# masapasa/qcpinn-convection-diffusion-qiskit

Hardware: AMD Instinct MI355X
Metric: collocation-points/sec (PDE+BC+IC loss step), 4-qubit cascade (higher is better)
Workload: dtype f32

## Files before the change

qcpinn-convection-diffusion-qiskit_amd/csrc/qc_circuit_reg_kernels.h:

```cpp
#pragma once
#include "qc_gates.h"
#include "qc_internal.h"

#include <stdlib.h>

#include <utility>

namespace {

template <int AB>
__device__ __forceinline__ bool qc_flag(int rt) {
  if constexpr (AB < 0) return rt != 0;
  else return AB != 0;
}

template <class T>
__device__ __forceinline__ const T* qc_launder(const T* p) {
  asm volatile("" : "+s"(p));
  return p;
}
template <class T>
__device__ __forceinline__ const __attribute__((address_space(4))) T* qc_const(const T* p) {
  return (const __attribute__((address_space(4))) T*)qc_launder(p);
}
// ... 11 lines not shown
__device__ __forceinline__ int64_t qc_opaque_s(int64_t v) {
  asm volatile("" : "+s"(v));
  return v;
}
__device__ __forceinline__ int qc_opaque_v(int v) {
  asm volatile("" : "+v"(v));
  return v;
}

template <int NQ>
struct DynProg {
  static constexpr int N = NQ;
  static constexpr bool lead_rx = true;
  __device__ static __forceinline__ int lead_slot(const QcGate* __restrict__ prog, int w) { return prog[w].slot; }
  template <int AB = -1, bool PIN = false>
  __device__ static __forceinline__ void fwd(SV<NQ> (&v)[1], const QcGate* __restrict__ prog,
                                             const QcTrig* __restrict__ trig, const float* __restrict__ umat,
                                             int n_gates, int absorb) {
    for (int g = qc_flag<AB>(absorb) ? NQ : 0; g < n_gates; ++g) {
      const QcGate gt = prog[g];
      const QcTrig tr = trig[g];
      qc_apply_gate<NQ, 1, false>(v, gt, tr.c, tr.s, umat);
    }
  }
  template <int AB = -1>
  __device__ static __forceinline__ void bwd(SV<NQ> (&cl)[2], const QcGate* __restrict__ prog,
                                             const QcTrig* __restrict__ trig, const float* __restrict__ umat,
                                             int n_gates, float* __restrict__ acc_wave, int lane, int absorb) {
    const int g_first = qc_flag<AB>(absorb) ? NQ : 0;
    for (int g = n_gates - 1; g >= g_first; --g) {
      const QcGate gt = prog[g];
      const QcTrig tr = trig[g];
      if (gt.op != QC_U4 && gt.slot >= 0) {
        const float gr = qc_wave_sum_to_lane63(qc_gate_grad<NQ>(cl[1], cl[0], gt));
        if (lane == 63) acc_wave[gt.slot] += gr;
      }
      qc_apply_gate<NQ, 2, true>(cl, gt, tr.c, tr.s, umat);
    }
  }
};

struct SGate {
  int op, ba, bb, slot;
};

template <int NQ, int K, bool ADJ, int OP, int BA, int BB, int SLOT>
__device__ __forceinline__ void qc_static_gate(SV<NQ> (&v)[K], const float c, const float s_in) {
  const float s = ADJ ? -s_in : s_in;
#pragma unroll
  for (int q = 0; q < K; ++q) {
    if constexpr (OP == QC_RX) g_rx<NQ, BA>(v[q], c, s);
    else if constexpr (OP == QC_RY) g_ry<NQ, BA>(v[q], c, s);
    else if constexpr (OP == QC_RZ) g_rz<NQ, BA>(v[q], c, s);
    else if constexpr (OP == QC_H) g_h<NQ, BA>(v[q]);
    else if constexpr (OP == QC_CNOT) g_cnot<NQ, BA, BB>(v[q]);
    else if constexpr (OP == QC_CRX) g_crx<NQ, BA, BB>(v[q], c, s);
    else if constexpr (OP == QC_CRZ) g_crz<NQ, BA, BB>(v[q], c, s);
  }
}

template <int NQ, int OP, int BA, int BB>
__device__ __forceinline__ float qc_static_grad(const SV<NQ>& lam, const SV<NQ>& chi) {
  if constexpr (OP == QC_RX) return ip_x<NQ, BA>(lam, chi);
  else if constexpr (OP == QC_RY) return ip_y<NQ, BA>(lam, chi);
  else if constexpr (OP == QC_RZ) return ip_z<NQ, BA>(lam, chi);
  else if constexpr (OP == QC_CRX) return ip_cx<NQ, BA, BB>(lam, chi);
  else if constexpr (OP == QC_CRZ) return ip_cz<NQ, BA, BB>(lam, chi);
// ... 33 lines not shown
    (load_one<Is, AB>(t, trig), ...);
    __builtin_amdgcn_sched_barrier(0);
  }
  static constexpr bool is_diag(int i) { return i >= 0 && i < SP::G && (SP::g[i].op == QC_RZ || SP::g[i].op == QC_CRZ); }
  static constexpr int run_begin(int i) { while (is_diag(i - 1)) --i; return i; }
  static constexpr int run_end(int i) { while (is_diag(i)) ++i; return i; }
  static constexpr bool fused(int i) { return is_diag(i) && run_end(i) - run_begin(i) >= 2; }
  static constexpr int run_ordinal(int i) {
    int r = 0;
    for (int g = 0; g < run_begin(i);) {
      if (!is_diag(g)) { ++g; continue; }
      const int e = run_end(g);
      if (e - g >= 2) ++r;
      g = e;
    }
    return r;
  }
  static_assert(run_ordinal(SP::G) <= QC_MAX_DIAG_RUNS, "more fused diagonal runs than the host records (qc_find_diag_runs)");
  template <int I, bool ADJ, int K, bool PIN = true>
  __device__ static __forceinline__ void apply_table(SV<N> (&v)[K], const QcTrig* __restrict__ trig) {
    constexpr int off = SP::G + run_ordinal(I) * (1 << N);
    auto run = [&](auto tab) {
#pragma unroll
      for (int k = 0; k < (1 << N); ++k) {
        const float dr = tab[k].c, di = ADJ ? -tab[k].s : tab[k].s;
#pragma unroll
        for (int q = 0; q < K; ++q) v[q].a[k] = qc_cmul(dr, di, v[q].a[k]);
      }
    };
    if constexpr (PIN) run(qc_const_at(trig, v[0]) + off);
    else run(trig + off);
  }
  template <int H, int E>
  __device__ static __forceinline__ void run_grads(const QcPk<(1 << N)>& t, float (&gacc)[SP::P > 0 ? SP::P : 1]) {
    if constexpr (H < E) {
      constexpr SGate g = SP::g[H];
      constexpr bool ctl = g.op == QC_CRZ;
      constexpr int tb = ctl ? g.bb : g.ba;
      constexpr int cb = ctl ? g.ba : -1;
      qf2 a2 = {0.f, 0.f};
#pragma unroll
      for (int j = 0; j < (1 << (N - 1)); ++j) {
        if (cb >= 1 && !((j >> (cb >= 1 ? cb - 1 : 0)) & 1)) continue;
        if (tb >= 1 && ((j >> (tb >= 1 ? tb - 1 : 0)) & 1)) a2 -= t.p[j];
        else a2 += t.p[j];
      }
      const float acc = tb == 0 ? a2.x - a2.y : (cb == 0 ? a2.y : a2.x + a2.y);
      if constexpr (g.slot >= 0) gacc[g.slot] += qc_wave_sum_to_lane63(acc);
      run_grads<H + 1, E>(t, gacc);
    }
  }
  template <int I, int K, bool ADJ, bool PIN = true>
  __device__ static __forceinline__ void gate(SV<N> (&v)[K], const Trig& t, const float* __restrict__ umat) {
    constexpr SGate g = SP::g[I];
    if constexpr (g.op == QC_U4) {
      constexpr int off = (g.slot * 2 + (ADJ ? 1 : 0)) * 32;
      if constexpr (PIN) {
        const CMat u = qc_const_at(umat, v[0]) + off;
#pragma unroll
        for (int q = 0; q < K; ++q) g_u4<N, g.ba, g.bb>(v[q], u);
      } else {
#pragma unroll
        for (int q = 0; q < K; ++q) g_u4<N, g.ba, g.bb>(v[q], umat + off);
      }
    } else {
      qc_static_gate<N, K, ADJ, g.op, g.ba, g.bb, g.slot>(v, t.c[I], t.s[I]);
    }
  }
  template <int I, int AB, bool PIN>
  __device__ static __forceinline__ void fwd_one(SV<N> (&v)[1], const Trig& t, const float* __restrict__ umat,
                                                 int absorb, const QcTrig* __restrict__ trig) {
    if constexpr (I < N) {
      if (qc_flag<AB>(absorb)) return;
    }
    if constexpr (fused(I)) {
      if constexpr (I == run_begin(I)) {
        apply_table<I, false, 1, PIN>(v, trig);
        __builtin_amdgcn_sched_barrier(0);
      }
    } else {
      gate<I, 1, false, PIN>(v, t, umat);
      __builtin_amdgcn_sched_barrier(0);
    }
  }
  template <int AB, bool PIN, int... Is>
  __device__ static __forceinline__ void fwd_all(SV<N> (&v)[1], const Trig& t, const float* __restrict__ umat,
                                                 int absorb, const QcTrig* __restrict__ trig,
                                                 std::integer_sequence<int, Is...>) {
    (fwd_one<Is, AB, PIN>(v, t, umat, absorb, trig), ...);
  }
  template <int AB = -1, bool PIN = false>
  __device__ static __forceinline__ void fwd(SV<N> (&v)[1], const QcGate* __restrict__, const QcTrig* __restrict__ trig,
                                             const float* __restrict__ umat, int, int absorb) {
    Trig t;
    if constexpr (PIN) load_all<AB>(t, qc_const(trig), std::make_integer_sequence<int, SP::G>{});
    else load_all<AB>(t, trig, std::make_integer_sequence<int, SP::G>{});
    fwd_all<AB, PIN>(v, t, umat, absorb, trig, std::make_integer_sequence<int, SP::G>{});
  }
  template <int J, int AB>
  __device__ static __forceinline__ void bwd_one(SV<N> (&cl)[2], const Trig& t, const float* __restrict__ umat,
                                                 float (&gacc)[SP::P > 0 ? SP::P : 1], int absorb,
                                                 const QcTrig* __restrict__ trig) {
    constexpr int I = SP::G - 1 - J;
    constexpr SGate g = SP::g[I];
    if constexpr (I < N) {
      if (qc_flag<AB>(absorb)) return;
    }
    if constexpr (fused(I)) {
      if constexpr (I == run_end(I) - 1) {
        QcPk<(1 << N)> tk;
#pragma unroll
        for (int k = 0; k < (1 << N); ++k) {
          const qf2 m = cl[1].a[k] * qc_swp(cl[0].a[k]);
          tk[k] = m.x - m.y;
        }
        run_grads<run_begin(I), run_end(I)>(tk, gacc);
        apply_table<I, true, 2>(cl, trig);
        __builtin_amdgcn_sched_barrier(0);
      }
    } else {
      if constexpr (g.op != QC_U4 && g.slot >= 0)
        gacc[g.slot] += qc_wave_sum_to_lane63(qc_static_grad<N, g.op, g.ba, g.bb>(cl[1], cl[0]));
      gate<I, 2, true>(cl, t, umat);
      __builtin_amdgcn_sched_barrier(0);
    }
  }
  template <int AB, int... Js>
  __device__ static __forceinline__ void bwd_all(SV<N> (&cl)[2], const Trig& t, const float* __restrict__ umat,
                                                 float (&gacc)[SP::P > 0 ? SP::P : 1], int absorb,
                                                 const QcTrig* __restrict__ trig, std::integer_sequence<int, Js...>) {
    (bwd_one<Js, AB>(cl, t, umat, gacc, absorb, trig), ...);
  }
  template <int AB = -1>
  __device__ static __forceinline__ void bwd(SV<N> (&cl)[2], const QcGate* __restrict__, const QcTrig* __restrict__ trig,
                                             const float* __restrict__ umat, int, float* __restrict__ acc_wave,
                                             int lane, int absorb) {
    float gacc[SP::P > 0 ? SP::P : 1];
#pragma unroll
    for (int k = 0; k < (SP::P > 0 ? SP::P : 1); ++k) gacc[k] = 0.f;
    Trig t;
    load_all<AB>(t, qc_const(trig), std::make_integer_sequence<int, SP::G>{});
    bwd_all<AB>(cl, t, umat, gacc, absorb, trig, std::make_integer_sequence<int, SP::G>{});
    const int k0 = qc_opaque_v(0);
    const bool last = qc_opaque_v(lane) == 63;
#pragma unroll
    for (int k = 0; k < SP::P; ++k)
      if (last) acc_wave[k0 + k] += gacc[k];
  }
};

template <int AB = -1>
__device__ __forceinline__ void qc_wire_sincos(float& c, float& s, const float* __restrict__ a, int64_t B, int64_t p, int w,
                                               const QcTrig* __restrict__ trig, int absorb) {
  const float h = 0.5f * (a[(int64_t)w * B + p] + (qc_flag<AB>(absorb) ? trig[w].th : 0.f));
  sincosf(h, &s, &c);
// ... 111 lines not shown
  SV<N> cl[2];
  {
    SV<N> v[1];
    build_channel<N, AB>(v[0], 0, angles, B, pc, ampl, trig, absorb);
    PG::template fwd<AB, true>(v, prog, trig, umat, n_gates, absorb);
    cl[0] = v[0];
  }
  float qb[N];
#pragma unroll
  for (int w = 0; w < N; ++w) qb[w] = live ? cot[(int64_t)w * B + pc] : 0.f;
  {
    QcPk<(1 << N)> d;
    qc_sign_sums<N>(d, qb);
#pragma unroll
    for (int k = 0; k < (1 << N); ++k) cl[1].a[k] = qc_dup(d[k]) * cl[0].a[k];
  }
  PG::template bwd<AB>(cl, prog, trig, umat, n_gates, smem + wave * n_params, lane, absorb);
  float T[N];
  if (ampl) {
#pragma unroll
    for (int w = 0; w < N; ++w) T[w] = 2.f * cl[1].a[w].x;
  } else {
    QcPk<(1 << N)> Q0, Q1, Q2;
    channel_series<N, AB>(Q0, Q1, Q2, 0, qc_launder(angles), B, pc, trig, absorb);
    qc_embed_ip<N>(T, cl[1], Q0);
  }
  if (live) {
#pragma unroll
    for (int w = 0; w < N; ++w) d_angles[(int64_t)w * B + p] = T[w];
  }
  if (qc_flag<AB>(absorb)) {
#pragma unroll
    for (int w = 0; w < N; ++w) {
      const float tot = qc_wave_sum_to_lane63(live ? T[w] : 0.f);
      if (lane == 63) smem[wave * n_params + (AB < 0 ? prog[w].slot : PG::lead_slot(prog, w))] += tot;
    }
  }
  __syncthreads();
  const int64_t tile = (int64_t)bid * WPB + wave;
  if (tile * 64 < B)
    for (int i = lane; i < n_params; i += 64) part[(row0 + tile) * part_stride + i] = smem[wave * n_params + i];
}

template <class PG>
__global__ void __launch_bounds__(256) k_value_bwd(const QcGate* __restrict__ prog, const QcTrig* __restrict__ trig,
                                                   const float* __restrict__ umat, int n_gates, int n_params,
                                                   const float* __restrict__ angles, const float* __restrict__ cot,
                                                   float* __restrict__ d_angles, float* __restrict__ part,
                                                   int64_t part_stride, int64_t row0, int64_t B, int amp) {
  k_value_bwd_body<PG, 4>(blockIdx.x, prog, trig, umat, n_gates, n_params, angles, cot, d_angles, part, part_stride, row0, B, amp);
}

template <int A2>
__device__ __forceinline__ int64_t qc_chi_pair(int ch, int k, int64_t p) {
  return ((((p >> 6) * 6 + ch) * (A2 / 2) + k) << 6) | (p & 63);
}
template <int N>
__device__ __forceinline__ void qc_chi_write(float* __restrict__ chi_store, int ch, int64_t p, const SV<N>& v) {
  qf2* cs = reinterpret_cast<qf2*>(chi_store);
#pragma unroll
  for (int k = 0; k < (1 << N); ++k) cs[qc_chi_pair<(2 << N)>(ch, k, p)] = v.a[k];
}
template <int N>
__device__ __forceinline__ void qc_chi_read(SV<N>& v, const float* __restrict__ chi_store, int ch, int64_t p) {
  const qf2* cs = reinterpret_cast<const qf2*>(chi_store);
#pragma unroll
  for (int k = 0; k < (1 << N); ++k) v.a[k] = cs[qc_chi_pair<(2 << N)>(ch, k, p)];
// ... 178 lines not shown
    } else if (ch <= 3) {
      qc_pull_ip1<N>(T, cl[1], da);
  #pragma unroll
      for (int w = 0; w < N; ++w) buf[(0 * N + w) * 64 + lane] = T[w];
      qc_pull_ip0<N>(T, cl[1]);
  #pragma unroll
      for (int w = 0; w < N; ++w) buf[(1 * N + w) * 64 + lane] = T[w];
    } else {
      qc_pull_ip2<N>(T, cl[1], da, dda);
  #pragma unroll
      for (int w = 0; w < N; ++w) buf[(0 * N + w) * 64 + lane] = T[w];
      qc_pull_ip1<N>(T, cl[1], da);
  #pragma unroll
      for (int w = 0; w < N; ++w) buf[(1 * N + w) * 64 + lane] = 2.f * T[w];
      qc_pull_ip0<N>(T, cl[1]);
  #pragma unroll
      for (int w = 0; w < N; ++w) buf[(2 * N + w) * 64 + lane] = T[w];
    }
    __syncthreads();
    auto at = [&](int wv, int slot, int w) { return s_chi[((wv * 3 + slot) * N + w) * 64 + lane]; };
  #pragma unroll
    for (int w = 0; w < N; ++w) {
      float r;
      if (ch == 0)
        r = ((at(0, 0, w) + at(1, 0, w)) + (at(2, 0, w) + at(3, 0, w))) + (at(4, 0, w) + at(5, 0, w));
      else if (ch == 1)
        r = at(1, 1, w);
      else if (ch <= 3)
        r = at(ch, 1, w) + at(ch + 2, 1, w);
      else
        r = at(ch, 2, w);
      if (live) abar[((int64_t)ch * N + w) * B + p] = r;
      if ((amp >> 1) && ch == 0) {
        const float tot = qc_wave_sum_to_lane63(live ? r : 0.f);
        if (lane == 63) s_acc[prog[w].slot] += tot;
      }
    }
    __syncthreads();
  }
  for (int i = threadIdx.x; i < n_params; i += 384) {
    float s = 0.f;
#pragma unroll
    for (int wv = 0; wv < 6; ++wv) s += s_acc[wv * n_params + i];
    part[(row0 + bid) * part_stride + i] = s;
  }
}

template <class PG, bool LOAD>
__global__ void __launch_bounds__(384, QC_JB_WAVES) k_jets_bwd(const QcGate* __restrict__ prog, const QcTrig* __restrict__ trig,
                                                  const float* __restrict__ umat, int n_gates, int n_params,
                                                  const float* __restrict__ ajets, const float* __restrict__ qbar,
                                                  float* __restrict__ abar, float* __restrict__ part,
                                                  int64_t part_stride, int64_t row0, int64_t B,
                                                  const float* __restrict__ chi_store, int amp) {
  k_jets_bwd_body<PG, LOAD>(blockIdx.x, prog, trig, umat, n_gates, n_params, ajets, qbar, abar, part, part_stride, row0, B, chi_store, amp);
}

struct QcPartRow {
  float* row;
  int n_params;
};
template <class PG, bool ABSORB, class ROW>
__device__ __forceinline__ void k_jets_bwd2_body(const int64_t bid, const QcGate* __restrict__ prog, const QcTrig* __restrict__ trig,
                                                   const float* __restrict__ umat, int n_gates, int n_params,
                                                   const float* __restrict__ ajets, const float* __restrict__ qbar,
                                                   float* __restrict__ abar, const ROW row_of, int64_t B,
                                                   const float* __restrict__ chi_store) {
// ... 103 lines not shown
      for (int w = 0; w < N; ++w) t_own[w] += T[w];
    } else if (ch <= 3) {
      qc_pull_ip1<N>(T, cl[1], da);
#pragma unroll
      for (int w = 0; w < N; ++w) t_own[w] += T[w];
      qc_pull_ip0<N>(T, cl[1]);
#pragma unroll
      for (int w = 0; w < N; ++w) t_a1[w] = T[w];
    } else {
      qc_pull_ip2<N>(T, cl[1], da, dda);
#pragma unroll
      for (int w = 0; w < N; ++w) t_own[w] += T[w];
      qc_pull_ip1<N>(T, cl[1], da);
#pragma unroll
      for (int w = 0; w < N; ++w) t_a1[w] = fmaf(2.f, T[w], t_a1[w]);
      qc_pull_ip0<N>(T, cl[1]);
      if (live) {
#pragma unroll
        for (int w = 0; w < N; ++w) abar[((int64_t)ch * N + w) * Bq + p] = T[w];
      }
    }
  }
  const int wt = wvf();
  if (live) {
#pragma unroll
    for (int w = 0; w < N; ++w) abar[((int64_t)(wt == 0 ? 1 : wt + 1) * N + w) * B + p] = t_a1[w];
  }
  if (wt != 0) {
#pragma unroll
    for (int w = 0; w < N; ++w) s_t0[((wt - 1) * N + w) * 64 + lane] = t_own[w];
  }
  __syncthreads();
  if (wt == 0) {
#pragma unroll
    for (int w = 0; w < N; ++w) {
      const float r = (t_own[w] + s_t0[w * 64 + lane]) + s_t0[(N + w) * 64 + lane];
      if (live) abar[(int64_t)w * B + p] = r;
      if constexpr (ABSORB) {
        const float tot = qc_wave_sum_to_lane63(live ? r : 0.f);
        if (lane == 63) s_acc[PG::lead_slot(prog, w)] += tot;
      }
    }
  }
  __syncthreads();
  const QcPartRow pr = row_of();
  float* __restrict__ row = pr.row;
  for (int i = threadIdx.x; i < pr.n_params; i += 192) row[i] = (s_acc[i] + s_acc[pr.n_params + i]) + s_acc[2 * pr.n_params + i];
}

template <class PG>
__global__ void __launch_bounds__(384) k_circ_fwd_both(const QcGate* __restrict__ prog, const QcTrig* __restrict__ trig,
                                                       const float* __restrict__ umat, int n_gates,
                                                       const float* __restrict__ ajets, float* __restrict__ qjets, int64_t Br,
                                                       float* __restrict__ chi_store, const float* __restrict__ angles,
                                                       float* __restrict__ expval, int64_t Bv, int amp, int n_val) {
  if ((int)blockIdx.x >= n_val) k_jets_fwd_body<PG>(blockIdx.x - n_val, prog, trig, umat, n_gates, ajets, qjets, Br, chi_store, amp);
  else k_value_fwd_body<PG, 6>(blockIdx.x, prog, trig, umat, n_gates, angles, expval, Bv, amp);
}

template <class PG>
__global__ void __launch_bounds__(384, QC_JB_WAVES) k_circ_bwd_both(
    const QcGate* __restrict__ prog, const QcTrig* __restrict__ trig, const float* __restrict__ umat, int n_gates, int n_params,
    const float* __restrict__ ajets, const float* __restrict__ qbar, float* __restrict__ abar, int64_t row0_r, int64_t Br,
    const float* __restrict__ chi_store, const float* __restrict__ angles, const float* __restrict__ cot,
    float* __restrict__ d_angles, int64_t row0_v, int64_t Bv, float* __restrict__ part, int64_t part_stride, int amp, int n_val) {
  if ((int)blockIdx.x >= n_val)
    k_jets_bwd_body<PG, true>(blockIdx.x - n_val, prog, trig, umat, n_gates, n_params, ajets, qbar, abar, part, part_stride, row0_r, Br,
                              chi_store, amp);
  else
    k_value_bwd_body<PG, 6>(blockIdx.x, prog, trig, umat, n_gates, n_params, angles, cot, d_angles, part, part_stride,
                            row0_v, Bv, amp);
}

struct QcBwdResArgs {
// ... 155 lines not shown
```

qcpinn-convection-diffusion-qiskit_amd/csrc/qc_common.h:

```cpp
#pragma once
#include <hip/hip_runtime.h>
#include <stdint.h>

#include "qc_types.h"

#define QC_NCH 6

#define QC_WAVE 64

static inline int qc_ceil_div(int64_t a, int64_t b) { return (int)((a + b - 1) / b); }

__host__ __device__ inline bool qc_is_diag_op(int op) { return op == 2  || op == 6 ; }

struct QcDiagRuns {
  int n;
  int g0[QC_MAX_DIAG_RUNS], g1[QC_MAX_DIAG_RUNS];
  const int* list;
};

inline void qc_find_diag_runs(qc_program* pg) {
  pg->n_diag_runs = 0;
  pg->d_diag_list = nullptr;
  if (pg->n_qubits > 5) return;
  for (int g = 0; g < pg->n_gates;) {
// ... 143 lines not shown
    }
    QcTrig t = {dr, di, 0.f, 0.f};
    trig[n_gates + r * A + k] = t;
  }
}

__device__ __forceinline__ float qc_wave_sum_to_lane63(float v) {
  v += __builtin_bit_cast(float, __builtin_amdgcn_update_dpp(0, __builtin_bit_cast(int, v), 0xB1, 0xF, 0xF, true));
  v += __builtin_bit_cast(float, __builtin_amdgcn_update_dpp(0, __builtin_bit_cast(int, v), 0x4E, 0xF, 0xF, true));
  v += __builtin_bit_cast(float, __builtin_amdgcn_update_dpp(0, __builtin_bit_cast(int, v), 0x141, 0xF, 0xF, true));
  v += __builtin_bit_cast(float, __builtin_amdgcn_update_dpp(0, __builtin_bit_cast(int, v), 0x140, 0xF, 0xF, true));
  v += __builtin_bit_cast(float, __builtin_amdgcn_update_dpp(0, __builtin_bit_cast(int, v), 0x142, 0xA, 0xF, false));
  v += __builtin_bit_cast(float, __builtin_amdgcn_update_dpp(0, __builtin_bit_cast(int, v), 0x143, 0xC, 0xF, false));
  return v;
}

template <int NV>
__device__ __forceinline__ void qc_wave_sum_multi_to_lane63(float (&v)[NV]) {
#define QC_DPP_STEP_(CTRL)                                                                                       \
  _Pragma("unroll") for (int k = 0; k < NV; ++k)                                                                 \
    v[k] += __builtin_bit_cast(float, __builtin_amdgcn_update_dpp(0, __builtin_bit_cast(int, v[k]), CTRL, 0xF, 0xF, true));
  QC_DPP_STEP_(0xB1) QC_DPP_STEP_(0x4E) QC_DPP_STEP_(0x141) QC_DPP_STEP_(0x140)
#undef QC_DPP_STEP_
#pragma unroll
  for (int k = 0; k < NV; ++k) asm volatile("" : "+v"(v[k]));
  asm volatile("s_nop 1");
#pragma unroll
  for (int k = 0; k < NV; ++k) asm volatile("v_add_f32_dpp %0, %0, %0 row_bcast:15 row_mask:0xa bank_mask:0xf" : "+v"(v[k]));
  if constexpr (NV < 3) asm volatile("s_nop 1");
#pragma unroll
  for (int k = 0; k < NV; ++k) asm volatile("v_add_f32_dpp %0, %0, %0 row_bcast:31 row_mask:0xc bank_mask:0xf" : "+v"(v[k]));
}

__device__ __forceinline__ float qc_wave_sum(float v) {
  v = qc_wave_sum_to_lane63(v);
  return __builtin_bit_cast(float, __builtin_amdgcn_readlane(__builtin_bit_cast(int, v), 63));
}
```

qcpinn-convection-diffusion-qiskit_amd/csrc/qc_mlp.hip:

```cpp
#include "qc_internal.h"
#include "qc_philox.h"
#include <tuple>

namespace {

__device__ __forceinline__ float qc_tanh(float x) {
  const float e = __expf(2.f * x);
  return 1.f - 2.f * __builtin_amdgcn_rcpf(e + 1.f);
}

typedef float mf2 __attribute__((ext_vector_type(2)));
__device__ __forceinline__ mf2 m_dup(const float a) { return (mf2){a, a}; }
__device__ __forceinline__ mf2 m_fma(const mf2 a, const mf2 b, const mf2 c) { return __builtin_elementwise_fma(a, b, c); }

__device__ __forceinline__ float analytic_u(float t, float x, float y) {
  const float dx = x - 0.5f, dy = y - 0.5f;
  return expf(-100.f * (dx * dx + dy * dy)) * expf(-t);
}
__device__ __forceinline__ float analytic_r(float t, float x, float y, float D, float vx, float vy) {
  const float u = analytic_u(t, x, y);
  const float dx = x - 0.5f, dy = y - 0.5f;
  const float ut = -u, ux = -200.f * dx * u, uy = -200.f * dy * u;
  const float uxx = (40000.f * dx * dx - 400.f) * u;
  const float uyy = (40000.f * dy * dy - 400.f) * u;
// ... 531 lines not shown

template <int N, int NCH>
__device__ __forceinline__ void post_cotangents(float (&gb)[NCH], float& gw4, const float (&g)[NCH],
                                                const float (&ub)[NCH], const float z, const float w4) {
  const float d1 = 1.f - z * z;
  gw4 = ub[0] * z;
  gb[0] = ub[0] * d1;
  if constexpr (NCH == 6) {
    const float d2 = -2.f * z * d1;
    const float d3 = -2.f * (d1 * d1 + z * d2);
    const float gx2 = g[2] * g[2], gy2 = g[3] * g[3];
    const float lin = ub[1] * g[1] + ub[2] * g[2] + ub[3] * g[3];
    gw4 += d1 * lin + ub[4] * (d2 * gx2 + d1 * g[4]) + ub[5] * (d2 * gy2 + d1 * g[5]);
    gb[0] += d2 * lin + ub[4] * (d3 * gx2 + d2 * g[4]) + ub[5] * (d3 * gy2 + d2 * g[5]);
    gb[1] = ub[1] * d1;
    gb[2] = ub[2] * d1 + 2.f * ub[4] * d2 * g[2];
    gb[3] = ub[3] * d1 + 2.f * ub[5] * d2 * g[3];
    gb[4] = ub[4] * d1;
    gb[5] = ub[5] * d1;
  }
#pragma unroll
  for (int c = 0; c < NCH; ++c) gb[c] *= w4;
}

template <int NCH>
__device__ __forceinline__ void expand_ub(float (&ub)[NCH], float ub0, float gsc, const QcPde& pde) {
  ub[0] = ub0;
  if constexpr (NCH == 6) {
    ub[1] = gsc * pde.c_t;
    ub[2] = gsc * pde.c_x;
    ub[3] = gsc * pde.c_y;
    ub[4] = -pde.d_xx * gsc;
    ub[5] = -pde.d_yy * gsc;
  }
}

__device__ __forceinline__ void learn_coefs(float (&cf)[QC_COEF_N], const float* __restrict__ prm, const QcLayout& L,
                                            const float (&base)[QC_COEF_N], const float (&scale)[QC_COEF_N]) {
  const float* __restrict__ pk = prm + (L.NP - QC_COEF_N);
#pragma unroll
  for (int k = 0; k < QC_COEF_N; ++k) cf[k] = fmaf(scale[k], pk[k], base[k]);
}
__device__ __forceinline__ void learn_columns(float* __restrict__ row, const QcLayout& L, const QcLearn* lr, const int z,
                                              const float (&scale)[QC_COEF_N], const float (&cf)[QC_COEF_N], const float gsc,
                                              const float (&u)[6], const int lane, const bool tile0) {
  float gv[QC_COEF_N] = {gsc * u[0], gsc * u[1], gsc * u[2], gsc * u[3], -gsc * u[4], -gsc * u[5], gsc * (u[0] * u[0] * u[0])};
  qc_wave_sum_multi_to_lane63<QC_COEF_N>(gv);
  if (lane == 63) {
#pragma unroll
    for (int k = 0; k < QC_COEF_N; ++k) row[L.NP - QC_COEF_N + k] = scale[k] == 0.f ? 0.f : scale[k] * gv[k];
    if (tile0) {
      float* hist = (&lr->hist)[z];
      const QcOptState* st = (&lr->st)[z];
      if (hist != nullptr && st != nullptr) {
        const int hi = st->step - st->hist_base;
        if (hi >= 0 && hi < (&lr->hist_cap)[z]) {
#pragma unroll
          for (int k = 0; k < QC_COEF_N; ++k) hist[(int64_t)hi * QC_COEF_N + k] = cf[k];
        }
      }
    }
  }
}
__device__ __forceinline__ int learn_late() {
  int z = 0;
#if defined(__HIP_DEVICE_COMPILE__)
// ... 639 lines not shown
  }
}

constexpr int QC_POST_VALUE_TPB = 1;

template <int N>
struct QcPostW {
  template <int K>
  struct Blk { static constexpr int count = K; float w3[K][N], b3[K], w4[K]; };
};
template <int N, int K>
__device__ __forceinline__ void post_blk_load(typename QcPostW<N>::template Blk<K>& w, const float* __restrict__ W3,
                                              const float* __restrict__ b3, const float* __restrict__ W4, const int m) {
  const float* __restrict__ p3 = W3 + m * N;
  const float* __restrict__ pb = b3 + m;
  const float* __restrict__ p4 = W4 + m;
#pragma unroll
  for (int j = 0; j < K; ++j)
#pragma unroll
    for (int i = 0; i < N; ++i) w.w3[j][i] = p3[j * N + i];
#pragma unroll
  for (int j = 0; j < K; ++j) w.b3[j] = pb[j];
#pragma unroll
  for (int j = 0; j < K; ++j) w.w4[j] = p4[j];
}
struct QcColW {
  template <int K>
  struct Blk { static constexpr int count = K; float c[K]; };
};
constexpr int qc_post_ub_a(int n) { return n == 3 ? 2 : (n <= 4 ? 4 : (n <= 8 ? 2 : 1)); }
constexpr bool qc_post_pf(int n) { return n <= 8; }
constexpr int qc_post_ub_vb(int n) { return n <= 8 ? 2 : 1; }

template <int N, int TPB, bool DATA = false, bool LEARN = false, bool BAL = false>
__device__ __forceinline__ void k_post_fused_value_body(const int64_t bid, const float* __restrict__ X,
                                                        const float* __restrict__ prm, QcLayout L, QcPde pde,
                                                        const float* __restrict__ qjets, float* __restrict__ out_u,
                                                        float* __restrict__ qbar, float* __restrict__ part,
                                                        int64_t part_stride, int64_t row0, int64_t B,
                                                        float* __restrict__ s_v, const float* __restrict__ tg = nullptr,
                                                        const QcBal* bl = nullptr) {
  constexpr int WPT = QC_MS / TPB, QPW = QC_MS / WPT;
  const int lane = threadIdx.x & 63;
  const int wave = __builtin_amdgcn_readfirstlane(threadIdx.x >> 6);
  const int slot = wave / WPT, wt = wave % WPT;
  const int64_t tile = bid * TPB + slot;
  const bool tile_ok = tile * 64 < B;
  const int64_t p = tile * 64 + lane;
  const bool live = p < B;
  const int64_t pc = live ? p : B - 1;
  float* s_g = s_v + (size_t)slot * (L.H + WPT) * 64;
  float* s_u = s_g + L.H * 64;
  float q[N];
#pragma unroll
  for (int i = 0; i < N; ++i) q[i] = qjets[(int64_t)i * B + pc];
  const float* W3 = prm + L.oW3;
  const float* b3 = prm + L.ob3;
  const float* W4 = prm + L.oW4;
  const int hq = (L.H + QC_MS - 1) / QC_MS;
  const int m0 = tile_ok ? wt * QPW * hq : 0;
  const int m1 = !tile_ok ? 0 : ((m0 + QPW * hq) < L.H ? (m0 + QPW * hq) : L.H);
  float up[QPW];
#pragma unroll
  for (int k = 0; k < QPW; ++k) {
    up[k] = 0.f;
    const int k0 = m0 + k * hq, k1 = (k0 + hq) < m1 ? (k0 + hq) : m1;
// ... 22 lines not shown
  else s_u[wt * 64 + lane] = QPW == 2 ? up[0] + up[1] : up[0];
  __syncthreads();
  if constexpr (WPT == 2) u = s_u[lane] + s_u[64 + lane];
  if constexpr (WPT == 4) u = (s_u[lane] + s_u[64 + lane]) + (s_u[128 + lane] + s_u[192 + lane]);
  u += prm[L.ob4];
  float* row = part + (row0 + tile) * part_stride;
  const bool seg_a = p < pde.n_seg_a;
  float target;
  if constexpr (DATA) {
    target = tg[pc];
  } else {
    const float t = X[pc * 3 + 0], x = X[pc * 3 + 1], y = X[pc * 3 + 2];
    target = value_target(pde, seg_a, t, x, y);
  }
  if constexpr (BAL) bal_weights<1>(pde, prm, L, bl);
  const float e = live ? u - target : 0.f;
  const float ub0 = (seg_a ? pde.w_val_a : pde.w_val_b) * e;
  if (wt == 0 && tile_ok) {
    const float la = qc_wave_sum_to_lane63(seg_a ? e * e * pde.inv_n_a : 0.f);
    const float lb = qc_wave_sum_to_lane63(seg_a ? 0.f : e * e * pde.inv_n_b);
    const float sb4 = qc_wave_sum_to_lane63(ub0);
    if (lane == 63) {
      row[L.NP + 0] = 0.f;
      row[L.NP + 1] = lb;
      row[L.NP + 2] = la;
      row[L.ob4] = sb4;
      if constexpr (LEARN) learn_zero_columns(row, L);
      if constexpr (BAL) bal_zero_columns(row, L);
    }
    if (live) out_u[p] = ub0;
  }
  float ub[1];
  expand_ub<1>(ub, ub0, 0.f, pde);
  qc_unit_blocks<QcColW, qc_post_ub_vb(N), false>(
      m0, m1,
      [&](auto& w, const int m) {
#pragma unroll
        for (int j = 0; j < std::remove_reference_t<decltype(w)>::count; ++j) w.c[j] = W4[m + j];
      },
      [&](const auto& w, const int m) {
        constexpr int K = std::remove_reference_t<decltype(w)>::count;
        float wg[K * (N + 2)];
#pragma unroll
        for (int j = 0; j < K; ++j) {
          const float g[1] = {0.f};
          float gb[1], gw4;
          post_cotangents<N, 1>(gb, gw4, g, ub, s_g[(m + j) * 64 + lane], w.c[j]);
          s_g[(m + j) * 64 + lane] = gb[0];
#pragma unroll
          for (int i = 0; i < N; ++i) wg[j * (N + 2) + i] = fmaf(gb[0], q[i], 0.f);
          wg[j * (N + 2) + N] = gb[0];
          wg[j * (N + 2) + N + 1] = gw4;
        }
        qc_wave_sum_multi_to_lane63<K * (N + 2)>(wg);
        if (lane == 63) {
#pragma unroll
          for (int j = 0; j < K; ++j) {
#pragma unroll
            for (int i = 0; i < N; ++i) row[L.oW3 + (m + j) * N + i] = wg[j * (N + 2) + i];
            row[L.ob3 + m + j] = wg[j * (N + 2) + N];
            row[L.oW4 + m + j] = wg[j * (N + 2) + N + 1];
          }
        }
      });
  __syncthreads();
  if (live) {
    const int mh = tile_ok ? L.H : 0;
    for (int i = wt; i < N; i += WPT) {
      float qb = 0.f;
      qc_unit_blocks<QcColW, 4, true>(
          0, mh,
          [&](auto& w, const int m) {
#pragma unroll
            for (int j = 0; j < std::remove_reference_t<decltype(w)>::count; ++j) w.c[j] = W3[(m + j) * N + i];
          },
          [&](const auto& w, const int m) {
            constexpr int K = std::remove_reference_t<decltype(w)>::count;
            float gbv[K];
#pragma unroll
            for (int j = 0; j < K; ++j) gbv[j] = s_g[(m + j) * 64 + lane];
#pragma unroll
            for (int j = 0; j < K; ++j) qb = fmaf(w.c[j], gbv[j], qb);
          });
      qbar[(int64_t)i * B + p] = qb;
    }
  }
}


template <int N> constexpr int QC_POST6_UB_A = qc_post_ub_a(N);
template <int N> constexpr bool QC_POST6_PF_A = qc_post_pf(N);
template <int N> constexpr int QC_POST6_UB_B = 1;
template <int N> constexpr bool QC_POST6_PF_B = false;

template <int N, bool DATA = false, bool COEF = false, bool LEARN = false, bool BAL = false>
__device__ __forceinline__ void k_post_fused6_body(const int64_t bid, const float* __restrict__ X, const float* __restrict__ prm,
// ... 114 lines not shown
    if (lane == 63) {
      row[L.NP + 0] = ls;
      row[L.NP + 1] = 0.f;
      row[L.NP + 2] = 0.f;
      row[L.ob4] = sb4;
      if constexpr (BAL) bal_zero_columns(row, L);
    }
    if constexpr (LEARN) learn_columns(row, L, lr, lz, lscale, cf, gsc, u, lane, tile == 0);
    if constexpr (OPC) {
      if (live) {
        out_u[p] = ub0;
        out_u[B + p] = gsc * cf[1];
        out_u[2 * B + p] = gsc * cf[2];
        out_u[3 * B + p] = gsc * cf[3];
        out_u[4 * B + p] = -cf[4] * gsc;
        out_u[5 * B + p] = -cf[5] * gsc;
      }
    } else if (live) {
      out_u[p] = ub0;
      out_res[p] = gsc;
    }
  }
  float ub[NCH];
  if constexpr (OPC) {
    ub[0] = ub0; ub[1] = gsc * cf[1]; ub[2] = gsc * cf[2]; ub[3] = gsc * cf[3]; ub[4] = -cf[4] * gsc; ub[5] = -cf[5] * gsc;
  } else {
    expand_ub<NCH>(ub, ub0, gsc, pde);
  }
  mf2 qb2[3][N];
#pragma unroll
  for (int cp = 0; cp < 3; ++cp)
#pragma unroll
    for (int i = 0; i < N; ++i) qb2[cp][i] = (mf2){0.f, 0.f};
  qc_unit_blocks<QcPostW<N>, QC_POST6_UB_B<N>, QC_POST6_PF_B<N>>(m0, m1, load_blk, [&](const auto& w, const int m) {
    constexpr int K = std::remove_reference_t<decltype(w)>::count;
    float wg[K * (N + 2)];
#pragma unroll
    for (int j = 0; j < K; ++j) {
      mf2 g2[3];
      preact(w.w3[j], w.b3[j], g2);
      const float g[NCH] = {0.f, g2[0].y, g2[1].x, g2[1].y, g2[2].x, g2[2].y};
      const float z = s_z[(m + j) * 64 + lane];
      float gb[NCH], gw4;
      post_cotangents<N, NCH>(gb, gw4, g, ub, z, w.w4[j]);
      const mf2 gb2[3] = {(mf2){gb[0], gb[1]}, (mf2){gb[2], gb[3]}, (mf2){gb[4], gb[5]}};
#pragma unroll
      for (int i = 0; i < N; ++i) {
        const mf2 w3 = m_dup(w.w3[j][i]);
        mf2 acc = gb2[0] * q2[0][i];
#pragma unroll
        for (int cp = 0; cp < 3; ++cp) {
          qb2[cp][i] = m_fma(w3, gb2[cp], qb2[cp][i]);
          if (cp > 0) acc = m_fma(gb2[cp], q2[cp][i], acc);
        }
        wg[j * (N + 2) + i] = acc.x + acc.y;
      }
      wg[j * (N + 2) + N] = gb[0];
      wg[j * (N + 2) + N + 1] = gw4;
    }
    qc_wave_sum_multi_to_lane63<K * (N + 2)>(wg);
    if (lane == 63) {
#pragma unroll
      for (int j = 0; j < K; ++j) {
#pragma unroll
        for (int i = 0; i < N; ++i) row[L.oW3 + (m + j) * N + i] = wg[j * (N + 2) + i];
        row[L.ob3 + m + j] = wg[j * (N + 2) + N];
        row[L.oW4 + m + j] = wg[j * (N + 2) + N + 1];
      }
    }
  });
  __syncthreads();
#pragma unroll
  for (int cp = 0; cp < 3; ++cp)
#pragma unroll
    for (int i = 0; i < N; ++i) {
      s_q[wave][(2 * cp) * N + i][lane] = qb2[cp][i].x;
      s_q[wave][(2 * cp + 1) * N + i][lane] = qb2[cp][i].y;
    }
  __syncthreads();
  if (live) {
    constexpr int NF = (NCH * N + QC_MS - 1) / QC_MS;
    if constexpr (NF <= 12) {
      float v[NF];
#pragma unroll
      for (int j = 0; j < NF; ++j) {
        const int f = wave + QC_MS * j, fc = f < NCH * N ? f : 0;
        v[j] = (s_q[0][fc][lane] + s_q[1][fc][lane]) + (s_q[2][fc][lane] + s_q[3][fc][lane]);
      }
#pragma unroll
      for (int j = 0; j < NF; ++j) {
        const int f = wave + QC_MS * j;
        if (f < NCH * N) qbar[(int64_t)f * B + p] = v[j];
      }
    } else {
      for (int f = wave; f < NCH * N; f += QC_MS)
        qbar[(int64_t)f * B + p] = (s_q[0][f][lane] + s_q[1][f][lane]) + (s_q[2][f][lane] + s_q[3][f][lane]);
    }
  }
}

constexpr int QC_POST_FUSED_MAXH = 128;

// ... 119 lines not shown
    for (int m = m0; m < m1; ++m) {
      float g[NCH], z, f[NCH];
      hidden(m, g, z, f);
      float ubw[NCH], gk[QC_KMAX];
#pragma unroll
      for (int c = 0; c < NCH; ++c) ubw[c] = 0.f;
#pragma unroll
      for (int k = 0; k < QC_KMAX; ++k) {
        gk[k] = 0.f;
        if (k < K) {
          const float w4 = w4k[k * H1 + m];
#pragma unroll
          for (int c = 0; c < NCH; ++c) {
            ubw[c] = fmaf(w4, ub[k][c], ubw[c]);
            gk[k] = fmaf(ub[k][c], f[c], gk[k]);
          }
        }
      }
      float gb[NCH], gw4;
      post_cotangents<N, NCH>(gb, gw4, g, ubw, z, 1.f);
      float wg[N + 1];
#pragma unroll
      for (int i = 0; i < N; ++i) {
        const float w3 = W3[m * N + i];
        float sum = 0.f;
#pragma unroll
        for (int c = 0; c < NCH; ++c) {
          qb[c][i] = fmaf(w3, gb[c], qb[c][i]);
          sum = fmaf(gb[c], q[c][i], sum);
        }
        wg[i] = sum;
      }
      wg[N] = gb[0];
      qc_wave_sum_multi_to_lane63<N + 1>(wg);
#pragma unroll
      for (int k = 0; k < QC_KMAX; ++k)
        if (k < K) gk[k] = qc_wave_sum_to_lane63(gk[k]);
      if (lane == 63) {
#pragma unroll
        for (int i = 0; i < N; ++i) row[L.oW3 + m * N + i] = wg[i];
        row[L.ob3 + m] = wg[N];
#pragma unroll
        for (int k = 0; k < QC_KMAX; ++k)
          if (k < K) rowk[k * H1 + m] = gk[k];
      }
    }
    if (threadIdx.x == 0) {
      for (int m = 0; m < L.H; ++m) row[L.oW4 + m] = 0.f;
      row[L.ob4] = 0.f;
    }
#pragma unroll
    for (int c = 0; c < NCH; ++c)
#pragma unroll
      for (int i = 0; i < N; ++i) s_buf[wave][c * N + i][lane] = qb[c][i];
    __syncthreads();
    if (live) {
      for (int f = wave; f < NCH * N; f += QC_MS)
        qbar[(int64_t)f * B + p] = (s_buf[0][f][lane] + s_buf[1][f][lane]) + (s_buf[2][f][lane] + s_buf[3][f][lane]);
    }
  }
}

template <int N, int MAP, bool RF>
__global__ void __launch_bounds__(256) k_pre_fwd_both(float* __restrict__ Xr, float* __restrict__ Xv,
                                                      const float* __restrict__ prm, QcLayout L, float* __restrict__ ajr,
                                                      float* __restrict__ ajv, int64_t Br, int64_t Bv, int n_val, QcDraw draw) {
  if ((int)blockIdx.x >= n_val) k_pre_fwd_body<N, 6, MAP>(blockIdx.x - n_val, Xr, prm, L, ajr, Br, &draw, Xr);
  else k_pre_fwd_value4<N, MAP, RF>(blockIdx.x, Xv, prm, L, ajv, Bv, &draw, Xv);
}

template <int N, int MAP>
__global__ void k_pre_bwd_both(const float* __restrict__ Xr, const float* __restrict__ Xv, const float* __restrict__ prm,
                               QcLayout L, const float* __restrict__ abr, const float* __restrict__ abv,
                               float* __restrict__ part, int64_t part_stride, int64_t row0_r, int64_t row0_v, int64_t Br,
// ... 433 lines not shown
  for (int m = m0; m < m1; ++m) {
    float g[NCH], z, f[NCH];
    hidden(m, g, z, f);
    float ubw[NCH], gk[QC_KMAX];
#pragma unroll
    for (int c = 0; c < NCH; ++c) ubw[c] = 0.f;
#pragma unroll
    for (int k = 0; k < QC_KMAX; ++k) {
      gk[k] = 0.f;
      if (k < K) {
        const float w4 = W4[k * L.H + m];
#pragma unroll
        for (int c = 0; c < NCH; ++c) {
          ubw[c] = fmaf(w4, ub[k][c], ubw[c]);
          gk[k] = fmaf(ub[k][c], f[c], gk[k]);
        }
      }
    }
    float gb[NCH], gw4;
    post_cotangents<N, NCH>(gb, gw4, g, ubw, z, 1.f);
    float wg[N + 1];
#pragma unroll
    for (int i = 0; i < N; ++i) {
      const float w3 = W3[m * N + i];
      float sum = 0.f;
#pragma unroll
      for (int c = 0; c < NCH; ++c) {
        qb[c][i] = fmaf(w3, gb[c], qb[c][i]);
        sum = fmaf(gb[c], q[c][i], sum);
      }
      wg[i] = sum;
    }
    wg[N] = gb[0];
    qc_wave_sum_multi_to_lane63<N + 1>(wg);
#pragma unroll
    for (int k = 0; k < QC_KMAX; ++k)
      if (k < K) gk[k] = qc_wave_sum_to_lane63(gk[k]);
    if (lane == 63) {
#pragma unroll
      for (int i = 0; i < N; ++i) row[L.oW3 + m * N + i] = wg[i];
      row[L.ob3 + m] = wg[N];
#pragma unroll
      for (int k = 0; k < QC_KMAX; ++k)
        if (k < K) row[L.oW4 + k * L.H + m] = gk[k];
    }
  }
  if constexpr (NCH == 1) __syncthreads();
#pragma unroll
  for (int c = 0; c < NCH; ++c)
#pragma unroll
    for (int i = 0; i < N; ++i) s_buf[wave][c * N + i][lane] = qb[c][i];
  __syncthreads();
  if (live) {
    for (int f = wave; f < NCH * N; f += QC_MS)
      qbar[(int64_t)f * B + p] = (s_buf[0][f][lane] + s_buf[1][f][lane]) + (s_buf[2][f][lane] + s_buf[3][f][lane]);
  }
}

int qc_mlp_post_system(const float* prm, QcLayout L, const QcSys& sys, QcPde pde, const float* qjets, const float* tg,
                       float* qbar, float* part, int64_t part_stride, int64_t row0, int64_t B, int nch, hipStream_t st) {
  static_assert(QC_SYS_K == QC_KMAX, "outputs of a system");
  if (sys.K < 1 || sys.K > QC_KMAX || L.H > 1024) return QC_ERR_UNSUPPORTED;
  const int tiles = qc_ceil_div(B, 64);
  return qc_dispatch_n<1, QC_MLP_NMAX>(L.n, [&](auto n) {
    auto launch = [&](auto c) {
      hipLaunchKernelGGL((k_post_system<n(), c()>), dim3(tiles), dim3(256), 0, st, prm, L, sys, pde, qjets, tg, qbar, part,
                         part_stride, row0, B);
    };
    if (nch == 6) launch(qc_int<6>{}); else launch(qc_int<1>{});
  });
}

static int post_learn(const float* prm, QcLayout L, QcPde pde, const float* qjets, float* out_u, float* qbar, float* part,
                      int64_t part_stride, int64_t row0, int64_t B, int nch, hipStream_t st, const QcTarget& tg) {
// ... 99 lines not shown
```

Measured before the change: 618.6 million.

## Merge multi-value wave reductions via DPP/permlane transpose-sum and batch fused-run grads

Adds a merged wave-sum routine that reduces many per-lane values at once by pairing registers with half-mirror/ror DPP masks and permlane16/32 swaps, so each result lands in a distinct home lane rather than all in lane 63. Post-MLP weight-gradient stores are rewritten to write from those home lanes in parallel. Fused diagonal-run gradient terms are batched into one multi-value reduction instead of a separate reduction per gate. The aim is fewer cross-lane instructions in the many small reductions on the gradient path, in exchange for hand-scheduled inline asm with manual hazard padding and scattered lane-dependent stores.

```diff
diff --git a/qcpinn-convection-diffusion-qiskit_amd/csrc/qc_circuit_reg_kernels.h b/qcpinn-convection-diffusion-qiskit_amd/csrc/qc_circuit_reg_kernels.h
--- a/qcpinn-convection-diffusion-qiskit_amd/csrc/qc_circuit_reg_kernels.h
+++ b/qcpinn-convection-diffusion-qiskit_amd/csrc/qc_circuit_reg_kernels.h
@@ -67,7 +67,7 @@
       const QcGate gt = prog[g];
       const QcTrig tr = trig[g];
       if (gt.op != QC_U4 && gt.slot >= 0) {
-        const float gr = qc_wave_sum_to_lane63(qc_gate_grad<NQ>(cl[1], cl[0], gt));
+        const float gr = qc_wave_sum6_to_lane63(qc_gate_grad<NQ>(cl[1], cl[0], gt));
         if (lane == 63) acc_wave[gt.slot] += gr;
       }
       qc_apply_gate<NQ, 2, true>(cl, gt, tr.c, tr.s, umat);
@@ -167,7 +167,7 @@
     else run(trig + off);
   }
   template <int H, int E>
-  __device__ static __forceinline__ void run_grads(const QcPk<(1 << N)>& t, float (&gacc)[SP::P > 0 ? SP::P : 1]) {
+  __device__ static __forceinline__ void run_terms(const QcPk<(1 << N)>& t, float (&term)[E - run_begin(E - 1)]) {
     if constexpr (H < E) {
       constexpr SGate g = SP::g[H];
       constexpr bool ctl = g.op == QC_CRZ;
@@ -180,10 +180,21 @@
         if (tb >= 1 && ((j >> (tb >= 1 ? tb - 1 : 0)) & 1)) a2 -= t.p[j];
         else a2 += t.p[j];
       }
-      const float acc = tb == 0 ? a2.x - a2.y : (cb == 0 ? a2.y : a2.x + a2.y);
-      if constexpr (g.slot >= 0) gacc[g.slot] += qc_wave_sum_to_lane63(acc);
-      run_grads<H + 1, E>(t, gacc);
-    }
+      term[H - run_begin(H)] = tb == 0 ? a2.x - a2.y : (cb == 0 ? a2.y : a2.x + a2.y);
+      run_terms<H + 1, E>(t, term);
+    }
+  }
+  template <int H, int E, int... Is>
+  __device__ static __forceinline__ void run_grads(const QcPk<(1 << N)>& t, float (&gacc)[SP::P > 0 ? SP::P : 1],
+                                                   std::integer_sequence<int, Is...>) {
+    float term[E - H];
+    run_terms<H, E>(t, term);
+    qc_wave_sum_multi_to_lane63<E - H>(term);
+    (run_add<H + Is>(gacc, term[Is]), ...);
+  }
+  template <int I>
+  __device__ static __forceinline__ void run_add(float (&gacc)[SP::P > 0 ? SP::P : 1], const float tot) {
+    if constexpr (SP::g[I].slot >= 0) gacc[SP::g[I].slot] += tot;
   }
   template <int I, int K, bool ADJ, bool PIN = true>
   __device__ static __forceinline__ void gate(SV<N> (&v)[K], const Trig& t, const float* __restrict__ umat) {
@@ -249,13 +260,13 @@
           const qf2 m = cl[1].a[k] * qc_swp(cl[0].a[k]);
           tk[k] = m.x - m.y;
         }
-        run_grads<run_begin(I), run_end(I)>(tk, gacc);
+        run_grads<run_begin(I), run_end(I)>(tk, gacc, std::make_integer_sequence<int, run_end(I) - run_begin(I)>{});
         apply_table<I, true, 2>(cl, trig);
         __builtin_amdgcn_sched_barrier(0);
       }
     } else {
       if constexpr (g.op != QC_U4 && g.slot >= 0)
-        gacc[g.slot] += qc_wave_sum_to_lane63(qc_static_grad<N, g.op, g.ba, g.bb>(cl[1], cl[0]));
+        gacc[g.slot] += qc_wave_sum6_to_lane63(qc_static_grad<N, g.op, g.ba, g.bb>(cl[1], cl[0]));
       gate<I, 2, true>(cl, t, umat);
       __builtin_amdgcn_sched_barrier(0);
     }
@@ -433,7 +444,7 @@
   if (qc_flag<AB>(absorb)) {
 #pragma unroll
     for (int w = 0; w < N; ++w) {
-      const float tot = qc_wave_sum_to_lane63(live ? T[w] : 0.f);
+      const float tot = qc_wave_sum6_to_lane63(live ? T[w] : 0.f);
       if (lane == 63) smem[wave * n_params + (AB < 0 ? prog[w].slot : PG::lead_slot(prog, w))] += tot;
     }
   }
@@ -678,7 +689,7 @@
         r = at(ch, 2, w);
       if (live) abar[((int64_t)ch * N + w) * B + p] = r;
       if ((amp >> 1) && ch == 0) {
-        const float tot = qc_wave_sum_to_lane63(live ? r : 0.f);
+        const float tot = qc_wave_sum6_to_lane63(live ? r : 0.f);
         if (lane == 63) s_acc[prog[w].slot] += tot;
       }
     }
@@ -848,14 +859,18 @@
   }
   __syncthreads();
   if (wt == 0) {
+    float tot[N];
 #pragma unroll
     for (int w = 0; w < N; ++w) {
       const float r = (t_own[w] + s_t0[w * 64 + lane]) + s_t0[(N + w) * 64 + lane];
       if (live) abar[(int64_t)w * B + p] = r;
-      if constexpr (ABSORB) {
-        const float tot = qc_wave_sum_to_lane63(live ? r : 0.f);
-        if (lane == 63) s_acc[PG::lead_slot(prog, w)] += tot;
-      }
+      tot[w] = live ? r : 0.f;
+    }
+    if constexpr (ABSORB) {
+      qc_wave_sum_merged<N>(tot);
+#pragma unroll
+      for (int w = 0; w < N; ++w)
+        if (lane == qc_wave_sum_home_lane(N, w)) s_acc[PG::lead_slot(prog, w)] += tot[qc_wave_sum_home_reg(N, w)];
     }
   }
   __syncthreads();
diff --git a/qcpinn-convection-diffusion-qiskit_amd/csrc/qc_common.h b/qcpinn-convection-diffusion-qiskit_amd/csrc/qc_common.h
--- a/qcpinn-convection-diffusion-qiskit_amd/csrc/qc_common.h
+++ b/qcpinn-convection-diffusion-qiskit_amd/csrc/qc_common.h
@@ -199,6 +199,143 @@
   for (int k = 0; k < NV; ++k) asm volatile("v_add_f32_dpp %0, %0, %0 row_bcast:31 row_mask:0xc bank_mask:0xf" : "+v"(v[k]));
 }
 
+__device__ __forceinline__ float qc_wave_sum6_to_lane63(float v) {
+  float t[1] = {v};
+  qc_wave_sum_multi_to_lane63<1>(t);
+  return t[0];
+}
+
+__host__ __device__ constexpr int qc_ws_chunk_len(int NV, int k) { return NV - k / 16 * 16 < 16 ? NV - k / 16 * 16 : 16; }
+__host__ __device__ constexpr bool qc_ws_merged(int NV, int k) { return qc_ws_chunk_len(NV, k) >= 3; }
+__host__ __device__ constexpr int qc_wave_sum_home_lane(int NV, int k) {
+  return qc_ws_merged(NV, k) ? 4 * (k % 16) + 3 * (k & 1) : 63;
+}
+__host__ __device__ constexpr bool qc_wave_sum_is_home(int lane) { return (lane & 3) == 3 * ((lane >> 2) & 1); }
+__host__ __device__ constexpr int qc_wave_sum_home_index(int lane) { return lane >> 2; }
+__host__ __device__ constexpr int qc_wave_sum_home_reg(int NV, int k) { return qc_ws_merged(NV, k) ? k / 16 * 16 : k; }
+
+enum : int { QC_WS_HM, QC_WS_HMM, QC_WS_ROR, QC_WS_RORM, QC_WS_SW16, QC_WS_SW32 };
+struct QcWsOp {
+  int kind, a, b, pad;
+};
+struct QcWsPlan {
+  QcWsOp op[32];
+  int n;
+};
+__host__ __device__ constexpr QcWsPlan qc_ws_plan(int n) {
+  QcWsOp prog[32] = {};
+  int np = 0;
+  for (int a = 0; a < n; a += 2) {
+    prog[np++] = {QC_WS_HM, a, a, 0};
+    if (a + 1 < n) prog[np++] = {QC_WS_HMM, a, a + 1, 0};
+  }
+  for (int a = 0; a < n; a += 4) {
+    prog[np++] = {QC_WS_ROR, a, a, 0};
+    if (a + 2 < n) prog[np++] = {QC_WS_RORM, a, a + 2, 0};
+  }
+  for (int a = 0; a < n; a += 8) prog[np++] = {QC_WS_SW16, a, a + 4 < n ? a + 4 : 1, 0};
+  prog[np++] = {QC_WS_SW32, 0, 8 < n ? 8 : (n <= 4 ? 2 : 1), 0};
+  QcWsPlan P = {};
+  int age[16] = {};
+  for (int r = 0; r < 16; ++r) age[r] = 99;
+  bool done[32] = {};
+  int pad = 0;
+  while (P.n < np) {
+    int pick = -1;
+    for (int i = 0; i < np && pick < 0; ++i) {
+      if (done[i]) continue;
+      const QcWsOp o = prog[i];
+      const bool swap = o.kind == QC_WS_SW16 || o.kind == QC_WS_SW32;
+      bool ok = true;
+      for (int j = 0; j < i; ++j)
+        if (!done[j] && (prog[j].a == o.a || prog[j].a == o.b || prog[j].b == o.a || prog[j].b == o.b)) ok = false;
+      if (age[o.b] < 2 || ((swap || o.a == o.b) && age[o.a] < 2)) ok = false;
+      if (ok) pick = i;
+    }
+    if (pick < 0) {
+      ++pad;
+      for (int r = 0; r < 16; ++r) ++age[r];
+      continue;
+    }
+    QcWsOp o = prog[pick];
+    const bool swap = o.kind == QC_WS_SW16 || o.kind == QC_WS_SW32;
+    o.pad = pad;
+    pad = 0;
+    done[pick] = true;
+    P.op[P.n++] = o;
+    for (int r = 0; r < 16; ++r) age[r] += swap ? 2 : 1;
+    age[o.a] = 0;
+    if (swap) age[o.b] = 1;
+  }
+  return P;
+}
+
+template <int NV, int C0, int I>
+__device__ __forceinline__ void qc_ws_emit(float (&v)[NV]) {
+  constexpr QcWsPlan P = qc_ws_plan(qc_ws_chunk_len(NV, C0));
+  if constexpr (I < P.n) {
+    constexpr QcWsOp o = P.op[I];
+    static_assert(o.pad >= 0 && o.pad <= 2, "a hazard is two wait states");
+    float& x = v[C0 + o.a];
+    float& y = v[C0 + o.b];
+#define QC_WS_ASM_(INS, ...)                                                   \
+  do {                                                                         \
+    if constexpr (o.pad == 0) asm volatile(INS : __VA_ARGS__);                 \
+    else if constexpr (o.pad == 1) asm volatile("s_nop 0\n\t" INS : __VA_ARGS__); \
+    else asm volatile("s_nop 1\n\t" INS : __VA_ARGS__);                        \
+  } while (0)
+    if constexpr (o.kind == QC_WS_HM)
+      QC_WS_ASM_("v_add_f32_dpp %0, %0, %0 row_half_mirror row_mask:0xf bank_mask:0xf", "+v"(x));
+    else if constexpr (o.kind == QC_WS_HMM)
+      QC_WS_ASM_("v_add_f32_dpp %0, %1, %1 row_half_mirror row_mask:0xf bank_mask:0xa", "+v"(x) : "v"(y));
+    else if constexpr (o.kind == QC_WS_ROR)
+      QC_WS_ASM_("v_add_f32_dpp %0, %0, %0 row_ror:8 row_mask:0xf bank_mask:0xf", "+v"(x));
+    else if constexpr (o.kind == QC_WS_RORM)
+      QC_WS_ASM_("v_add_f32_dpp %0, %1, %1 row_ror:8 row_mask:0xf bank_mask:0xc", "+v"(x) : "v"(y));
+    else if constexpr (o.kind == QC_WS_SW16)
+      QC_WS_ASM_("v_permlane16_swap_b32 %0, %1\n\tv_add_f32 %0, %0, %1", "+v"(x), "+v"(y));
+    else
+      QC_WS_ASM_("v_permlane32_swap_b32 %0, %1\n\tv_add_f32 %0, %0, %1", "+v"(x), "+v"(y));
+#undef QC_WS_ASM_
+    qc_ws_emit<NV, C0, I + 1>(v);
+  }
+}
+template <int NV, int C0>
+__device__ __forceinline__ void qc_ws_chunks(float (&v)[NV]) {
+  if constexpr (C0 < NV) {
+    if constexpr (qc_ws_merged(NV, C0)) {
+      qc_ws_emit<NV, C0, 0>(v);
+    } else {
+      constexpr int R = NV - C0;
+      float t[R];
+#pragma unroll
+      for (int k = 0; k < R; ++k) t[k] = v[C0 + k];
+      qc_wave_sum_multi_to_lane63<R>(t);
+#pragma unroll
+      for (int k = 0; k < R; ++k) v[C0 + k] = t[k];
+    }
+    qc_ws_chunks<NV, C0 + 16>(v);
+  }
+}
+template <int NV>
+__device__ __forceinline__ void qc_wave_sum_merged(float (&v)[NV]) {
+  if constexpr (NV < 3) {
+    qc_wave_sum_multi_to_lane63<NV>(v);
+  } else {
+    constexpr int NM = NV - (qc_ws_merged(NV, NV - 1) ? 0 : NV % 16);
+#pragma unroll
+    for (int k = 0; k < NM; ++k)
+      v[k] += __builtin_bit_cast(float, __builtin_amdgcn_update_dpp(0, __builtin_bit_cast(int, v[k]), 0xB1, 0xF, 0xF, true));
+#pragma unroll
+    for (int k = 0; k < NM; ++k)
+      v[k] += __builtin_bit_cast(float, __builtin_amdgcn_update_dpp(0, __builtin_bit_cast(int, v[k]), 0x4E, 0xF, 0xF, true));
+#pragma unroll
+    for (int k = 0; k < NM; ++k) asm volatile("" : "+v"(v[k]));
+    asm volatile("s_nop 1");
+    qc_ws_chunks<NV, 0>(v);
+  }
+}
+
 __device__ __forceinline__ float qc_wave_sum(float v) {
   v = qc_wave_sum_to_lane63(v);
   return __builtin_bit_cast(float, __builtin_amdgcn_readlane(__builtin_bit_cast(int, v), 63));
diff --git a/qcpinn-convection-diffusion-qiskit_amd/csrc/qc_mlp.hip b/qcpinn-convection-diffusion-qiskit_amd/csrc/qc_mlp.hip
--- a/qcpinn-convection-diffusion-qiskit_amd/csrc/qc_mlp.hip
+++ b/qcpinn-convection-diffusion-qiskit_amd/csrc/qc_mlp.hip
@@ -587,6 +587,21 @@
     ub[3] = gsc * pde.c_y;
     ub[4] = -pde.d_xx * gsc;
     ub[5] = -pde.d_yy * gsc;
+  }
+}
+
+template <int N, int C = 0>
+__device__ __forceinline__ void post_store_w3b3(float* __restrict__ row, const QcLayout& L, const float (&wg)[N + 1], const int m,
+                                                const int lane) {
+  if constexpr (C * 16 < N + 1) {
+    if constexpr (qc_ws_merged(N + 1, C * 16)) {
+      const int r = C * 16 + qc_wave_sum_home_index(lane);
+      if (qc_wave_sum_is_home(lane) && r <= N) row[r < N ? L.oW3 + m * N + r : L.ob3 + m] = wg[C * 16];
+    } else if (lane == 63) {
+#pragma unroll
+      for (int r = C * 16; r <= N; ++r) row[r < N ? L.oW3 + m * N + r : L.ob3 + m] = wg[r];
+    }
+    post_store_w3b3<N, C + 1>(row, L, wg, m, lane);
   }
 }
 
@@ -1292,6 +1307,45 @@
 constexpr bool qc_post_pf(int n) { return n <= 8; }
 constexpr int qc_post_ub_vb(int n) { return n <= 8 ? 2 : 1; }
 
+template <int N, int KMAX>
+struct QcPostCols {
+  static constexpr int NC = (KMAX * (N + 2) + 15) / 16;
+  unsigned col0[NC], cstep[NC];
+  bool home;
+  __device__ __forceinline__ QcPostCols(const QcLayout& L, const int lane) {
+    home = qc_wave_sum_is_home(lane);
+#pragma unroll
+    for (int c = 0; c < NC; ++c) {
+      const int k = 16 * c + qc_wave_sum_home_index(lane), j = k / (N + 2), r = k % (N + 2);
+      col0[c] = r < N ? L.oW3 + j * N + r : (r == N ? L.ob3 : L.oW4) + j;
+      cstep[c] = r < N ? N : 1;
+    }
+  }
+  template <int K>
+  __device__ __forceinline__ void store(float* __restrict__ row, const QcLayout& L, const float (&wg)[K * (N + 2)], const int m,
+                                        const int lane) const {
+    static_assert(K <= KMAX, "columns formed for KMAX units");
+    store_chunk<K, 0>(row, L, wg, m, lane);
+  }
+  template <int K, int C>
+  __device__ __forceinline__ void store_chunk(float* __restrict__ row, const QcLayout& L, const float (&wg)[K * (N + 2)],
+                                              const int m, const int lane) const {
+    constexpr int NV = K * (N + 2);
+    if constexpr (C * 16 < NV) {
+      if constexpr (qc_ws_merged(NV, C * 16)) {
+        if (home && 16 * C + qc_wave_sum_home_index(lane) < NV) row[col0[C] + __umul24(m, cstep[C])] = wg[qc_wave_sum_home_reg(NV, C * 16)];
+      } else if (lane == 63) {
+#pragma unroll
+        for (int k = C * 16; k < NV; ++k) {
+          const int j = k / (N + 2), r = k % (N + 2);
+          row[r < N ? L.oW3 + (m + j) * N + r : (r == N ? L.ob3 : L.oW4) + m + j] = wg[k];
+        }
+      }
+      store_chunk<K, C + 1>(row, L, wg, m, lane);
+    }
+  }
+};
+
 template <int N, int TPB, bool DATA = false, bool LEARN = false, bool BAL = false>
 __device__ __forceinline__ void k_post_fused_value_body(const int64_t bid, const float* __restrict__ X,
                                                         const float* __restrict__ prm, QcLayout L, QcPde pde,
@@ -1380,6 +1434,7 @@
   }
   float ub[1];
   expand_ub<1>(ub, ub0, 0.f, pde);
+  const QcPostCols<N, qc_post_ub_vb(N)> cols(L, lane);
   qc_unit_blocks<QcColW, qc_post_ub_vb(N), false>(
       m0, m1,
       [&](auto& w, const int m) {
@@ -1400,16 +1455,8 @@
           wg[j * (N + 2) + N] = gb[0];
           wg[j * (N + 2) + N + 1] = gw4;
         }
-        qc_wave_sum_multi_to_lane63<K * (N + 2)>(wg);
-        if (lane == 63) {
-#pragma unroll
-          for (int j = 0; j < K; ++j) {
-#pragma unroll
-            for (int i = 0; i < N; ++i) row[L.oW3 + (m + j) * N + i] = wg[j * (N + 2) + i];
-            row[L.ob3 + m + j] = wg[j * (N + 2) + N];
-            row[L.oW4 + m + j] = wg[j * (N + 2) + N + 1];
-          }
-        }
+        qc_wave_sum_merged<K * (N + 2)>(wg);
+        cols.template store<K>(row, L, wg, m, lane);
       });
   __syncthreads();
   if (live) {
@@ -1590,6 +1637,7 @@
   for (int cp = 0; cp < 3; ++cp)
 #pragma unroll
     for (int i = 0; i < N; ++i) qb2[cp][i] = (mf2){0.f, 0.f};
+  const QcPostCols<N, QC_POST6_UB_B<N>> cols(L, lane);
   qc_unit_blocks<QcPostW<N>, QC_POST6_UB_B<N>, QC_POST6_PF_B<N>>(m0, m1, load_blk, [&](const auto& w, const int m) {
     constexpr int K = std::remove_reference_t<decltype(w)>::count;
     float wg[K * (N + 2)];
@@ -1616,16 +1664,8 @@
       wg[j * (N + 2) + N] = gb[0];
       wg[j * (N + 2) + N + 1] = gw4;
     }
-    qc_wave_sum_multi_to_lane63<K * (N + 2)>(wg);
-    if (lane == 63) {
-#pragma unroll
-      for (int j = 0; j < K; ++j) {
-#pragma unroll
-        for (int i = 0; i < N; ++i) row[L.oW3 + (m + j) * N + i] = wg[j * (N + 2) + i];
-        row[L.ob3 + m + j] = wg[j * (N + 2) + N];
-        row[L.oW4 + m + j] = wg[j * (N + 2) + N + 1];
-      }
-    }
+    qc_wave_sum_merged<K * (N + 2)>(wg);
+    cols.template store<K>(row, L, wg, m, lane);
   });
   __syncthreads();
 #pragma unroll
@@ -1811,14 +1851,12 @@
         wg[i] = sum;
       }
       wg[N] = gb[0];
-      qc_wave_sum_multi_to_lane63<N + 1>(wg);
+      qc_wave_sum_merged<N + 1>(wg);
+      post_store_w3b3<N>(row, L, wg, m, lane);
 #pragma unroll
       for (int k = 0; k < QC_KMAX; ++k)
         if (k < K) gk[k] = qc_wave_sum_to_lane63(gk[k]);
       if (lane == 63) {
-#pragma unroll
-        for (int i = 0; i < N; ++i) row[L.oW3 + m * N + i] = wg[i];
-        row[L.ob3 + m] = wg[N];
 #pragma unroll
         for (int k = 0; k < QC_KMAX; ++k)
           if (k < K) rowk[k * H1 + m] = gk[k];
@@ -2318,14 +2356,12 @@
       wg[i] = sum;
     }
     wg[N] = gb[0];
-    qc_wave_sum_multi_to_lane63<N + 1>(wg);
+    qc_wave_sum_merged<N + 1>(wg);
+    post_store_w3b3<N>(row, L, wg, m, lane);
 #pragma unroll
     for (int k = 0; k < QC_KMAX; ++k)
       if (k < K) gk[k] = qc_wave_sum_to_lane63(gk[k]);
     if (lane == 63) {
-#pragma unroll
-      for (int i = 0; i < N; ++i) row[L.oW3 + m * N + i] = wg[i];
-      row[L.ob3 + m] = wg[N];
 #pragma unroll
       for (int k = 0; k < QC_KMAX; ++k)
         if (k < K) row[L.oW4 + k * L.H + m] = gk[k];
```

New measurement: 632.8 million (median of 6 runs). 1.02x the previous value.
